# jnetter6/RRTQX_3D

Measured on NVIDIA B200. Metric: kd_range_queries_per_s, higher is better.
Workload: dtype f64

## Files before the change

### rrtqx_3d_b200/csrc/range_fused.cuh

```cuda

constexpr int FUSED_TAB = 256;
constexpr int FUSED_ROUNDS = 4;
#ifndef FUSED_U
#define FUSED_U 4
#endif

__device__ __forceinline__ void sts32(unsigned addr, int v) {
  asm volatile("st.shared.b32 [%0], %1;" ::"r"(addr), "r"(v) : "memory");
}
__device__ __forceinline__ int lds32(unsigned addr) {
  int v;
  asm volatile("ld.shared.b32 %0, [%1];" : "=r"(v) : "r"(addr) : "memory");
  return v;
}
__device__ __forceinline__ unsigned pin_reg(unsigned v) {
  unsigned r;
  asm volatile("mov.u32 %0, %1;" : "=r"(r) : "r"(v));
  return r;
}

#ifdef RRTQX_LEGACY
template <int D, int QN>
struct Group {
  double q[QN][D];
// ... 396 lines not shown
  const double *dT = nullptr;
  if (dr) {
    res->tq.ensure((size_t)nq, st);
    thresh_kernel<<<div_up(nq, 256), 256, 0, st>>>(dr, nq, res->tq.p);
    post_launch(ctx);
    dT = res->tq.p;
  }
  size_t cap = count_only ? 0 : res->idx.cap;
  if (!count_only && want_dist) cap = std::min(cap, res->dist.cap);
  if (!count_only && cap == 0) {
    cap = (size_t)nq * 64;
    res->idx.ensure(cap, st, 0, 1.0);
    if (want_dist) res->dist.ensure(cap, st, 0, 1.0);
    cap = want_dist ? std::min(res->idx.cap, res->dist.cap) : res->idx.cap;
  }
  double k_est = 1e9;
  if (!dr && r > 0.0 && std::isfinite(r)) {
    double vol = 1.0;
    int dims = 0;
    const int nd[3] = {t->nx, t->ny, t->nz};
    for (int c = 0; c < 3; ++c)
      if (nd[c] > 1) { vol *= nd[c] * t->cell[c]; dims++; }
    const double ball = dims == 3 ? 4.18879 * r * r * r : (dims == 2 ? 3.14159 * r * r : 2.0 * r);
    k_est = dims ? 1.15 * (double)t->n * ball / vol : (double)t->n;
  } else if (!dr) {
    k_est = 0.0;
  }
  int variant = k_est <= 576.0 ? 0 : (k_est <= 1280.0 ? 1 : (k_est <= 2048.0 ? 2 : 3));
  if (ctx->tune.fused_variant >= 0) variant = ctx->tune.fused_variant;
#ifdef RRTQX_LEGACY
  const int kernel_gen = ctx->tune.range_kernel;
#endif
  unsigned long long total = 0;
  for (int attempt = 0; attempt < 2; ++attempt) {
    GridView g = t->view();
    RQ_CUDA(cudaMemsetAsync(res->cursor.p, 0, 4 * sizeof(unsigned long long), st));
    {
      PhaseScope p2(ctx, "range_fill");
#ifdef RRTQX_LEGACY
#define RQ_FUSED(NW_, CAP_)                                                                                          \
  launch_fused<D, NW_, CAP_>(ctx, g, dq, res->qbins > 0 ? res->qsorted.p : nullptr, res->qorder.p, nq, r, T, dr, dT, res->counts.p, res->offsets.p, res->idx.p, \
                             want_dist ? res->dist.p : nullptr, (unsigned long long)cap, res->cursor.p,             \
                             count_only ? 0 : 1)
#endif
#define RQ_V5(NW_, CAP_, TAB_)                                                                                       \
  launch_v5<D, NW_, CAP_, TAB_>(ctx, g, kq, kqs, korder, knq, r, T, dr, dT, kcounts, koffsets, res->idx.p, \
                                want_dist ? res->dist.p : nullptr, (unsigned long long)cap, res->cursor.p, count_only ? 0 : 1, ghost ? 1 : 0)
#ifdef RRTQX_LEGACY
      if (kernel_gen >= 5 || ghost)
#endif
      {
        const int v5_nw = ctx->tune.v5_nw;
#ifdef RRTQX_EXPERIMENT
        if (variant == 0 && v5_nw == 32) RQ_V5(32, 704, 256);
        else
#endif
        if (variant == 0 && v5_nw == 28) RQ_V5(28, 704, 256);
        else if (variant == 0 && v5_nw == 20) RQ_V5(20, 704, 256);
        else if (variant == 0) RQ_V5(24, 704, 256);
        else if (variant == 1) RQ_V5(24, 1408, 512);
        else if (variant == 2) RQ_V5(16, 2176, 1024);
        else RQ_V5(8, 4224, 2048);
      }
#ifdef RRTQX_LEGACY
      else
      if (variant == 0) RQ_FUSED(28, 576);
      else if (variant == 1) RQ_FUSED(20, 1280);
      else if (variant == 2) RQ_FUSED(12, 2048);
      else RQ_FUSED(6, 4096);
#undef RQ_FUSED
#endif
#undef RQ_V5
    }
    RQ_CUDA(cudaMemcpyAsync(&total, res->cursor.p, sizeof(total), cudaMemcpyDeviceToHost, st));
    RQ_CUDA(cudaStreamSynchronize(st));
    if (count_only || total <= cap) break;
    RQ_REQUIRE(attempt == 0, "internal: range output did not fit after resizing");
    cap = (size_t)total + (size_t)(total / 32) + 1024;
    res->idx.ensure(cap, st, 0, 1.0);
    if (want_dist) res->dist.ensure(cap, st, 0, 1.0);
    cap = want_dist ? std::min(res->idx.cap, res->dist.cap) : res->idx.cap;
  }
  if (ghost) {
    ghost_merge_kernel<<<div_up(nq, 256), 256, 0, st>>>(res->vcounts.p, res->voffsets.p, nq, res->counts.p, res->offsets.p);
    post_launch(ctx);
  }
  res->n_queries = nq;
  res->total = (int64_t)total;
  res->has_lists = !count_only;
  res->has_dist = !count_only && want_dist;
}
```

### rrtqx_3d_b200/csrc/range_v5.cuh

```cuda

constexpr int V5_TABPAD = 16;
constexpr int V5_UNIT = 128;
constexpr int V5_RING = 64;
#ifndef V5_U_TRIPS
#define V5_U_TRIPS 4
#endif
constexpr int V5_U = V5_U_TRIPS;

__device__ __forceinline__ unsigned long long pk2(float a, float b) {
  unsigned long long r;
  asm("mov.b64 %0, {%1, %2};" : "=l"(r) : "f"(a), "f"(b));
  return r;
}
__device__ __forceinline__ void upk2(unsigned long long r, float &a, float &b) {
  asm("mov.b64 {%0, %1}, %2;" : "=f"(a), "=f"(b) : "l"(r));
}
__device__ __forceinline__ unsigned long long fma2(unsigned long long a, unsigned long long b, unsigned long long c) {
  unsigned long long r;
  asm("fma.rn.f32x2 %0, %1, %2, %3;" : "=l"(r) : "l"(a), "l"(b), "l"(c));
  return r;
}
__device__ __forceinline__ unsigned long long sub2(unsigned long long a, unsigned long long b) {
  unsigned long long r;
  asm("sub.rn.f32x2 %0, %1, %2;" : "=l"(r) : "l"(a), "l"(b));
// ... 67 lines not shown
  auto visit = [&](bool valid, int node, double px, double py, double pz, double pw) {
    const double s = sqdist<D>(q, px, py, pz, pw);
    const bool hit = valid && (s < T);
    const unsigned m = __ballot_sync(FULL, hit);
    if (WRITE && hit) {
      const int64_t o = base + cnt + __popc(m & lt);
      out_idx[o] = node;
      if (out_dist) out_dist[o] = __dsqrt_rn(s);
    }
    cnt += __popc(m);
  };
  if (g.n_sorted > 0 && r > 0.0) {
    const double r_infl = r * (1.0 + 1e-9);
    const double r2_infl = r_infl * r_infl;
    const int cy0 = cell_of(q[1] - r_infl, g.lo[1], g.inv[1], g.ny);
    const int cy1 = cell_of(q[1] + r_infl, g.lo[1], g.inv[1], g.ny);
    const int cz0 = D >= 3 ? cell_of(q[2] - r_infl, g.lo[2], g.inv[2], g.nz) : 0;
    const int cz1 = D >= 3 ? cell_of(q[2] + r_infl, g.lo[2], g.inv[2], g.nz) : 0;
    const int wy = cy1 - cy0 + 1;
    const int nrows = wy * (cz1 - cz0 + 1);
    for (int rb = 0; rb < nrows; rb += 32) {
      RowSpan sp{0, 0};
      const int row = rb + lane;
      if (row < nrows) sp = row_span<D>(g, q, r_infl, r2_infl, cy0 + row % wy, cz0 + row / wy);
      const int lim = min(32, nrows - rb);
      for (int t = 0; t < lim; ++t) {
        const int a = __shfl_sync(FULL, sp.start, t);
        const int b = __shfl_sync(FULL, sp.end, t);
        for (int j0 = a; j0 < b; j0 += 32) {
          const int j = j0 + lane;
          const bool v = j < b;
          double4 p = make_double4(0, 0, 0, 0);
          int node = 0;
          if (v) {
            p = g.d4[j];
            node = D <= 3 ? (int)__double_as_longlong(p.w) : g.sperm[j];
          }
          visit(v, node, p.x, p.y, p.z, p.w);
        }
      }
    }
  }
  if (r > 0.0)
    for (int j0 = g.n_sorted; j0 < g.n_total; j0 += 32) {
      const int j = j0 + lane;
      const bool v = j < g.n_total;
      double4 p = make_double4(0, 0, 0, 0);
      if (v) p = g.pos[j];
      visit(v, j, p.x, p.y, p.z, p.w);
    }
  return cnt;
}

template <int D, bool TAIL>
__device__ __forceinline__ void v5_flush(const GridView &g, const double *q, unsigned sbuf_k, unsigned stab, int n, int lane,
                                         int32_t *__restrict__ oi, double *__restrict__ od) {
#ifndef V5_FLUSH_U
#define V5_FLUSH_U 4
#endif
  constexpr int U = V5_FLUSH_U;
  auto fetch = [&](unsigned h, int &node, double4 &p) {
    if (!TAIL || !(h & 0x8000u)) {
      const int ent = lds32(stab + 4u * (h >> 3));
      const int slot = (ent >> 4) + (int)(h & 7u);
      p = ldg256(g.d4 + slot);
      node = D <= 3 ? (int)__double_as_longlong(p.w) : g.sperm[slot];
    } else {
      node = g.n_sorted + (int)(h & 0x7fffu);
      p = g.pos[node];
    }
  };
  const int n_full = (n / (32 * U)) * (32 * U);
  for (int h0 = lane; h0 < n_full; h0 += 32 * U) {
    int node[U];
    double4 p[U];
#pragma unroll
    for (int u = 0; u < U; ++u) fetch(lds16(sbuf_k + 2u * (unsigned)(h0 + 32 * u)), node[u], p[u]);
#pragma unroll
    for (int u = 0; u < U; ++u) {
      v5_st(oi + h0 + 32 * u, node[u]);
      if (od) v5_st(od + h0 + 32 * u, __dsqrt_rn(sqdist<D>(q, p[u].x, p[u].y, p[u].z, p[u].w)));
    }
  }
  auto tail = [&](auto rows_tag) {
    constexpr int R = decltype(rows_tag)::value;
    const int h0 = n_full + lane;
    int node[R];
    double4 p[R];
#pragma unroll
    for (int u = 0; u < R; ++u) {
      const int hh = h0 + 32 * u < n ? h0 + 32 * u : 0;
      fetch(lds16(sbuf_k + 2u * (unsigned)hh), node[u], p[u]);
    }
#pragma unroll
    for (int u = 0; u < R; ++u)
      if (h0 + 32 * u < n) {
        v5_st(oi + h0 + 32 * u, node[u]);
        if (od) v5_st(od + h0 + 32 * u, __dsqrt_rn(sqdist<D>(q, p[u].x, p[u].y, p[u].z, p[u].w)));
      }
  };
  const int rem = n - n_full;
  if (U >= 4 && rem > 64) tail(std::integral_constant<int, (U >= 4 ? 4 : 1)>{});
  else if (rem > 32) tail(std::integral_constant<int, 2>{});
  else if (rem > 0) tail(std::integral_constant<int, 1>{});
}

template <int D>
__device__ __noinline__ void v5_flush_tail(const GridView *gp, const double *qs, unsigned sbuf_k, unsigned stab, int n,
                                           int32_t *__restrict__ oi, double *__restrict__ od) {
  double q[D];
#pragma unroll
  for (int c = 0; c < D; ++c) q[c] = qs[c];
  v5_flush<D, true>(*gp, q, sbuf_k, stab, n, lane_id(), oi, od);
}

struct V5Radius {
  float rf, r2f;
  float Tm;
  float cM1, cM0;
  float sum_max;
  bool live;
};
__host__ __device__ __forceinline__ V5Radius v5_radius(double r, double T, bool have) {
  V5Radius R;
  R.live = have && (r > 0.0);
  const double ri = r * (1.0 + 1e-9);
  R.rf = f32_up(ri) * (1.0f + 1e-6f);
  R.r2f = f32_up(ri * ri) * (1.0f + 1e-5f);
  float Tm, M;
  bool ex;
  v5_filter(T, 0.0f, Tm, M, ex);
  const float Tf = f32_up(T), sT = sqrtf(Tf);
  R.Tm = Tm;
  R.cM0 = M;
  R.cM1 = 12.0f * (sT * 1.000001f) * 6.03e-8f * 1.000001f;
  R.sum_max = ex ? -1.0f : sT * 0.999999f * (1.0f / (1024.0f * 6.03e-8f)) * 0.99999f;
  if (!R.live) { R.Tm = -INFINITY; R.r2f = -1.0f; R.cM0 = 0.0f; R.cM1 = 0.0f; R.sum_max = INFINITY; }
  return R;
}

struct V5Params {
  V5Radius RU;
  float invx, invy, invz, celly, cellz;
  unsigned unit;
  int ghost_pairs;
};

__device__ __forceinline__ int clampi_fast(float v, int n) { return min(max(__float2int_rd(v), 0), n - 1); }

__device__ __forceinline__ float sqrt_approx(float x) {
  float y;
  asm("sqrt.approx.f32 %0, %1;" : "=f"(y) : "f"(x));
  return y;
}

template <int D, int NW, int CAP, int TAB, bool UNIFORM>
__global__ void __launch_bounds__(NW * 32, 1)
range_v5_kernel(GridView g_param, V5Params P, const double *__restrict__ queries, const double *__restrict__ qsorted,
                const int32_t *__restrict__ qorder, int64_t nq, double r_uniform, double T_uniform,
                const double *__restrict__ ranges, const double *__restrict__ Tq, int32_t *__restrict__ counts,
                int64_t *__restrict__ offsets, int32_t *__restrict__ out_idx, double *__restrict__ out_dist,
                unsigned long long cap, unsigned long long *__restrict__ cursor, int write_lists) {
  extern __shared__ int s_buf[];
  __shared__ GridView s_g;
  __shared__ unsigned s_ticket;
  __shared__ unsigned s_pub[V5_RING];
  __shared__ long long s_base[V5_RING];
  const GridView &g = g_param;
  if (threadIdx.x == 0) { s_g = g_param; s_ticket = 0; }
  if (threadIdx.x < V5_RING) s_pub[threadIdx.x] = 0;
  __syncthreads();
  const int lane = lane_id(), warp = threadIdx.x >> 5;
  const unsigned lt = lanemask_lt();
  const unsigned s0 = (unsigned)__cvta_generic_to_shared(s_buf);
  const unsigned sbuf = pin_reg(s0 + 2u * (unsigned)(warp * 2 * CAP));
  const unsigned stab = pin_reg(s0 + 2u * (unsigned)(NW * 2 * CAP) + 4u * (unsigned)(warp * (TAB + V5_TABPAD)));
  const float &invx = P.invx, &invy = P.invy, &invz = P.invz, &celly = P.celly, &cellz = P.cellz;
  const float fmaxabs = g.n_sorted > 0 ? *g.fmaxabs : 0.0f;
  const bool has_tail = g.n_total > g.n_sorted;
  const unsigned grp = pin_reg((unsigned)lane >> 3), sub = pin_reg((unsigned)lane & 7u);
  constexpr bool uniform = UNIFORM;

  const int64_t n_pairs = (nq + 1) >> 1;
  for (;;) {
    {
      unsigned tk = 0;
      if (lane == 0) tk = atomicAdd(&s_ticket, 1u);
      tk = __shfl_sync(FULL, tk, 0);
      const unsigned unit = tk / P.unit, off = tk - unit * P.unit, slot = unit % V5_RING;
      long long base = 0;
      if (lane == 0) {
        if (off == 0) {
          base = (long long)atomicAdd(&cursor[1], (unsigned long long)P.unit);
          s_base[slot] = base;
          __threadfence_block();
          atomicExch(&s_pub[slot], unit + 1u);
        } else {
          while (atomicAdd(&s_pub[slot], 0u) != unit + 1u) __nanosleep(32);
          base = *(volatile long long *)&s_base[slot];
        }
      }
      base = __shfl_sync(FULL, base, 0);
      if (base >= n_pairs) break;
      const int64_t qfirst = (base + off) * 2;
      if (qfirst >= nq) continue;
      const bool have1 = qfirst + 1 < nq;
      const int qid0 = qorder[qfirst], qid1 = have1 ? qorder[qfirst + 1] : -1;
      const double *qs0 = qsorted ? qsorted + qfirst * D : queries + (int64_t)qid0 * D;
      const double *qs1 = !have1 ? qs0 : (qsorted ? qs0 + D : queries + (int64_t)qid1 * D);
      V5Radius Rq0, Rq1;
      if (!uniform) {
        Rq0 = v5_radius(ranges[qid0], Tq[qid0], true);
        Rq1 = have1 ? v5_radius(ranges[qid1], Tq[qid1], true) : Rq0;
      }
      const V5Radius &R0 = uniform ? P.RU : Rq0, &R1 = uniform ? P.RU : Rq1;
      auto fp32_query = [&](const double *qs, float (&qf)[4], float &mab) {
        mab = 0.0f;
#pragma unroll
        for (int c = 0; c < 4; ++c) {
          if (c < D) {
            const double v = qs[c];
            qf[c] = __double2float_rn(c < 3 ? __dsub_rn(v, g.lo[c < 3 ? c : 0]) : v);
            mab = fmaxf(mab, fabsf(qf[c]));
          } else {
            qf[c] = 0.0f;
          }
        }
#pragma unroll
        for (int c = 0; c < D; ++c) if (qf[c] != qf[c]) mab = -1.0f;
      };
      auto exactT = [&](int k) { return uniform ? T_uniform : ((k == 0 || !have1) ? Tq[qid0] : Tq[qid1]); };
      auto exactR = [&](int k) { return uniform ? r_uniform : ((k == 0 || !have1) ? ranges[qid0] : ranges[qid1]); };

      int root_extra = 0;
      {
        const double4 p0 = g.pos[0];
        double q0[D], q1[D];
#pragma unroll
        for (int c = 0; c < D; ++c) { q0[c] = qs0[c]; q1[c] = qs1[c]; }
        const double T0 = exactT(0), T1 = exactT(1);
        const double sr0 = sqdist<D>(q0, p0.x, p0.y, p0.z, p0.w), sr1 = sqdist<D>(q1, p0.x, p0.y, p0.z, p0.w);
        if (!(sr0 < T0) && sr0 <= T0 * 1.000001 && __dsqrt_rn(sr0) <= exactR(0)) root_extra |= 1;
        if (have1 && !P.ghost_pairs && !(sr1 < T1) && sr1 <= T1 * 1.000001 && __dsqrt_rn(sr1) <= exactR(1)) root_extra |= 2;
      }
      const bool live0 = R0.live, live1 = R1.live;
      bool exact_path = false;
      int n_ent = 0;
      if (live0 || live1) {
        float qf0[4], qf1[4], mab0, mab1;
        fp32_query(qs0, qf0, mab0);
        fp32_query(qs1, qf1, mab1);
        const bool rows0 = live0 && !(mab0 < 0.0f), rows1 = live1 && !(mab1 < 0.0f);
        exact_path = (rows0 && !(fmaxabs + mab0 <= R0.sum_max)) || (rows1 && !(fmaxabs + mab1 <= R1.sum_max));
        if (!exact_path && g.n_sorted > 0 && (rows0 || rows1)) {
          float ff0[3], ff1[3];
          ff0[0] = qf0[0] * invx; ff0[1] = qf0[1] * invy; ff0[2] = D >= 3 ? qf0[2] * invz : 0.0f;
          ff1[0] = qf1[0] * invx; ff1[1] = qf1[1] * invy; ff1[2] = D >= 3 ? qf1[2] * invz : 0.0f;
          const float ry0 = R0.rf * invy + 1e-3f, ry1 = R1.rf * invy + 1e-3f;
          const float rz0 = R0.rf * invz + 1e-3f, rz1 = R1.rf * invz + 1e-3f;
          int cy0 = 0x7fffffff, cy1 = -1, cz0 = 0, cz1 = 0;
          if (D >= 3) { cz0 = 0x7fffffff; cz1 = -1; }
          if (rows0) {
            cy0 = clampi_fast(ff0[1] - ry0, g.ny); cy1 = clampi_fast(ff0[1] + ry0, g.ny);
            if (D >= 3) { cz0 = clampi_fast(ff0[2] - rz0, g.nz); cz1 = clampi_fast(ff0[2] + rz0, g.nz); }
          }
          if (rows1) {
            cy0 = min(cy0, clampi_fast(ff1[1] - ry1, g.ny)); cy1 = max(cy1, clampi_fast(ff1[1] + ry1, g.ny));
            if (D >= 3) { cz0 = min(cz0, clampi_fast(ff1[2] - rz1, g.nz)); cz1 = max(cz1, clampi_fast(ff1[2] + rz1, g.nz)); }
          }
          const int wy = cy1 - cy0 + 1;
          const int sh = 32 - __clz(wy - 1);
          const int nslots = (cz1 - cz0 + 1) << sh;
          for (int rb = 0; rb < nslots; rb += 32) {
            int sa_ = 0, sb_ = 0;
            const int slot = rb + lane;
            const int ry = slot & ((1 << sh) - 1);
            if (slot < nslots && ry < wy) {
              const int cy = cy0 + ry, cz = cz0 + (slot >> sh);
              const float ylo = cy == 0 ? -INFINITY : (float)cy, yhi = cy == g.ny - 1 ? INFINITY : (float)(cy + 1);
              const float zlo = cz == 0 ? -INFINITY : (float)cz, zhi = cz == g.nz - 1 ? INFINITY : (float)(cz + 1);
              int ca = 0x7fffffff, cb = -1;
              auto span = [&](const float *ff, float r2f) {
                float dy = fmaxf(fmaxf(ylo - ff[1], ff[1] - yhi) * (1.0f - 1e-6f) - 1e-3f, 0.0f) * celly;
                float rem = r2f - dy * dy;
                if (D >= 3) {
                  float dz = fmaxf(fmaxf(zlo - ff[2], ff[2] - zhi) * (1.0f - 1e-6f) - 1e-3f, 0.0f) * cellz;
                  rem -= dz * dz;
                }
                if (rem >= 0.0f) {
                  const float xc = sqrt_approx(rem) * (1.0f + 1e-5f) * invx + 1e-3f;
                  ca = min(ca, clampi_fast(ff[0] - xc, g.nx));
                  cb = max(cb, clampi_fast(ff[0] + xc, g.nx));
                }
              };
              if (rows0) span(ff0, R0.r2f);
              if (rows1) span(ff1, R1.r2f);
              if (cb >= ca) {
                const int rbase = (cz * g.ny + cy) * g.nx;
                sa_ = g.cell_start[rbase + ca];
                sb_ = g.cell_start[rbase + cb + 1];
              }
            }
            const int todo = (sb_ - sa_ + 7) >> 3;
            int incl = todo;
#pragma unroll
            for (int o = 1; o < 32; o <<= 1) {
              const int t = __shfl_up_sync(FULL, incl, o);
              if (lane >= o) incl += t;
            }
            const int sum = __shfl_sync(FULL, incl, 31);
            if (n_ent + sum > TAB) {
              exact_path = true;
              break;
            }
            unsigned ta = stab + 4u * (unsigned)(n_ent + incl - todo);
            for (int i = 0; i < todo; ++i) {
              sts32(ta, (sa_ << 4) | min(8, sb_ - sa_));
              ta += 4u;
              sa_ += 8;
            }
            n_ent += sum;
          }
        }
      }
      int cnt0 = 0, cnt1 = 0;
      bool overflow = false;
      if (exact_path) {
        cnt0 = live0 ? v5_exact_query<D, false>(&s_g, qs0, exactT(0), exactR(0), 0, nullptr, nullptr) : 0;
        cnt1 = (live1 && have1) ? v5_exact_query<D, false>(&s_g, qs1, exactT(1), exactR(1), 0, nullptr, nullptr) : 0;
        overflow = true;
      } else if (live0 || live1) {
        float qf0[4], qf1[4], mab0, mab1;
        fp32_query(qs0, qf0, mab0);
        fp32_query(qs1, qf1, mab1);
        const unsigned long long qx2 = pk2(qf0[0], qf1[0]), qy2 = pk2(qf0[1], qf1[1]);
        const unsigned long long qz2 = pk2(qf0[2], qf1[2]), qw2 = pk2(qf0[3], qf1[3]);
        const unsigned long long nT2 = pk2(-R0.Tm, -R1.Tm);
        const float M = fmaxf(R0.cM1 * (fmaxabs + mab0) + R0.cM0, R1.cM1 * (fmaxabs + mab1) + R1.cM0) * 1.000001f;
        unsigned wp0 = sbuf, wp1 = sbuf + 2u * CAP;
        const unsigned lim0 = sbuf + 2u * (CAP - 32 * V5_U), lim1 = sbuf + 2u * (2 * CAP - 32 * V5_U);

        const unsigned goff = 4u * grp;
        const unsigned hv0 = (grp << 3) | sub;
        int jj[V5_U];
        float4 c[V5_U];
        const int dummy = g.n_sorted + 7;
        auto load_group = [&](unsigned tb) {
          const unsigned taddr = tb + goff;
#pragma unroll
          for (int u = 0; u < V5_U; ++u) {
            const int ent = lds32(taddr + 16u * u);
            jj[u] = sub < (unsigned)(ent & 15) ? (ent >> 4) + (int)sub : dummy;
          }
#pragma unroll
          for (int u = 0; u < V5_U; ++u) {
            c[u] = g.f4[jj[u]];
          }
        };
        auto test_group = [&](auto store_tag, unsigned tb, bool more) {
          constexpr bool STORE = decltype(store_tag)::value;
          const unsigned hv = hv0 + ((tb - stab) << 1);
          float sa[V5_U], sb[V5_U];
          int jc[V5_U];
          float band = INFINITY;
#pragma unroll
          for (int u = 0; u < V5_U; ++u) {
            unsigned long long s2 = sub2(qx2, pk2(c[u].x, c[u].x));
            s2 = fma2(s2, s2, nT2);
            unsigned long long d2 = sub2(qy2, pk2(c[u].y, c[u].y));
            s2 = fma2(d2, d2, s2);
            if (D >= 3) { d2 = sub2(qz2, pk2(c[u].z, c[u].z)); s2 = fma2(d2, d2, s2); }
            if (D >= 4) { d2 = sub2(qw2, pk2(c[u].w, c[u].w)); s2 = fma2(d2, d2, s2); }
            upk2(s2, sa[u], sb[u]);
            band = fminf(band, fminf(fabsf(sa[u]), fabsf(sb[u])));
            jc[u] = jj[u];
          }
          if (more) load_group(tb + 4u * 4 * V5_U);
          if (__any_sync(FULL, band <= M)) {
            double qa[D], qb[D];
#pragma unroll
            for (int cc = 0; cc < D; ++cc) { qa[cc] = qs0[cc]; qb[cc] = qs1[cc]; }
            const double Ta = exactT(0), Tb = exactT(1);
#pragma unroll
            for (int u = 0; u < V5_U; ++u) {
              if (sa[u] < INFINITY || sb[u] < INFINITY) {
                const double4 p = g.d4[jc[u]];
                sa[u] = (live0 && sqdist<D>(qa, p.x, p.y, p.z, p.w) < Ta) ? -INFINITY : INFINITY;
                sb[u] = (live1 && sqdist<D>(qb, p.x, p.y, p.z, p.w) < Tb) ? -INFINITY : INFINITY;
              }
            }
          }
#pragma unroll
          for (int u = 0; u < V5_U; ++u) {
            const bool h0 = sa[u] < M;
            const unsigned m0 = __ballot_sync(FULL, h0);
            if (STORE && h0) sts16(wp0 + 2u * __popc(m0 & lt), hv + 32u * u);
            wp0 += 2u * __popc(m0);
            const bool h1 = sb[u] < M;
            const unsigned m1 = __ballot_sync(FULL, h1);
            if (STORE && h1) sts16(wp1 + 2u * __popc(m1 & lt), hv + 32u * u);
            wp1 += 2u * __popc(m1);
          }
        };
        if (n_ent > 0) {
          if (lane < V5_TABPAD) sts32(stab + 4u * (unsigned)(n_ent + lane), 0);
          __syncwarp();
          unsigned tb = stab;
          const unsigned tend = stab + 4u * (unsigned)n_ent;
          load_group(tb);
          while (tb < tend && wp0 <= lim0 && wp1 <= lim1) {
            const unsigned nb = tb + 4u * 4 * V5_U;
            test_group(std::true_type{}, tb, nb < tend);
            tb = nb;
          }
          if (tb < tend) {
            overflow = true;
            do {
              const unsigned nb = tb + 4u * 4 * V5_U;
              test_group(std::false_type{}, tb, nb < tend);
              tb = nb;
            } while (tb < tend);
          }
          __syncwarp();
        }
        if (has_tail && g.n_total - g.n_sorted > 0x8000) overflow = true;
        if (has_tail) {
          double qa[D], qb[D];
#pragma unroll
          for (int cc = 0; cc < D; ++cc) { qa[cc] = qs0[cc]; qb[cc] = qs1[cc]; }
          const double Ta = exactT(0), Tb = exactT(1);
          for (int j0 = g.n_sorted; j0 < g.n_total; j0 += 32) {
            const int j = j0 + lane;
            const bool v = j < g.n_total;
            double4 p = make_double4(0, 0, 0, 0);
            if (v) p = g.pos[j];
            const bool h0 = v && live0 && (sqdist<D>(qa, p.x, p.y, p.z, p.w) < Ta);
            const bool h1 = v && live1 && (sqdist<D>(qb, p.x, p.y, p.z, p.w) < Tb);
            const unsigned m0 = __ballot_sync(FULL, h0);
            const unsigned o0 = wp0 + 2u * __popc(m0 & lt);
            if (h0 && o0 < sbuf + 2u * CAP) sts16(o0, 0x8000u | (unsigned)((j - g.n_sorted) & 0x7fff));
            wp0 += 2u * __popc(m0);
            const unsigned m1 = __ballot_sync(FULL, h1);
            const unsigned o1 = wp1 + 2u * __popc(m1 & lt);
            if (h1 && o1 < sbuf + 4u * CAP) sts16(o1, 0x8000u | (unsigned)((j - g.n_sorted) & 0x7fff));
            wp1 += 2u * __popc(m1);
          }
        }
        cnt0 = (int)((wp0 - sbuf) >> 1);
        cnt1 = (int)((wp1 - (sbuf + 2u * CAP)) >> 1);
        if (cnt0 > CAP || cnt1 > CAP) overflow = true;
      }
      const bool live1w = live1 && have1;
      if (!have1) cnt1 = 0;

      const int tot0 = cnt0 + (root_extra & 1), tot1 = cnt1 + ((root_extra >> 1) & 1);
      unsigned long long b0 = 0;
      if (lane == 0) b0 = atomicAdd(&cursor[0], (unsigned long long)(tot0 + tot1));
      b0 = __shfl_sync(FULL, b0, 0);
      if (lane == 0) {
        counts[qid0] = tot0;
        offsets[qid0] = (int64_t)b0;
        if (have1) {
          counts[qid1] = tot1;
          offsets[qid1] = (int64_t)(b0 + (unsigned long long)tot0);
        }
      }
      if (!write_lists || b0 + (unsigned long long)(tot0 + tot1) > cap) continue;
      __syncwarp();
      auto emit = [&](int k, const double *qs, int cnt, int64_t base, bool live_k) {
        if (!live_k) return;
        if (overflow) {
          v5_exact_query<D, true>(&s_g, qs, exactT(k), exactR(k), base, out_idx, out_dist);
        } else {
          const unsigned sb_k = sbuf + 2u * (unsigned)(k * CAP);
          if (has_tail) {
            v5_flush_tail<D>(&s_g, qs, sb_k, stab, cnt, out_idx + base, out_dist ? out_dist + base : nullptr);
          } else {
            double q[D];
#pragma unroll
            for (int c = 0; c < D; ++c) q[c] = qs[c];
            v5_flush<D, false>(g, q, sb_k, stab, cnt, lane, out_idx + base, out_dist ? out_dist + base : nullptr);
          }
        }
      };
#pragma unroll 1
      for (int k = 0; k < 2; ++k)
        emit(k, k ? qs1 : qs0, k ? cnt1 : cnt0, (int64_t)b0 + (k ? tot0 : 0), k ? live1w : live0);
      if (root_extra && lane == 0) {
        const double4 p0 = g.pos[0];
        if (root_extra & 1) {
          double q[D];
#pragma unroll
          for (int c = 0; c < D; ++c) q[c] = qs0[c];
          out_idx[b0 + cnt0] = 0;
          if (out_dist) out_dist[b0 + cnt0] = __dsqrt_rn(sqdist<D>(q, p0.x, p0.y, p0.z, p0.w));
        }
        if (root_extra & 2) {
          double q[D];
#pragma unroll
          for (int c = 0; c < D; ++c) q[c] = qs1[c];
          out_idx[b0 + tot0 + cnt1] = 0;
          if (out_dist) out_dist[b0 + tot0 + cnt1] = __dsqrt_rn(sqdist<D>(q, p0.x, p0.y, p0.z, p0.w));
        }
      }
      __syncwarp();
    }
  }
}

template <int D>
__global__ void ghost_expand_kernel(WrapInfo wrap, const double *__restrict__ queries, const double *__restrict__ qsorted,
                                    const int32_t *__restrict__ qorder, int64_t nq, double r,
                                    double *__restrict__ vq, int32_t *__restrict__ vorder) {
  const int64_t j = (int64_t)blockIdx.x * blockDim.x + threadIdx.x;
  if (j >= nq) return;
  const int qid = qorder[j];
  const double *src = qsorted ? qsorted + j * D : queries + (int64_t)qid * D;
  double q[D], gh[D];
#pragma unroll
  for (int k = 0; k < D; ++k) q[k] = src[k];
  const bool used = make_ghost<D>(wrap, q, 1, r, gh);
#pragma unroll
  for (int k = 0; k < D; ++k) {
    vq[(2 * j) * D + k] = q[k];
    vq[(2 * j + 1) * D + k] = used ? gh[k] : __longlong_as_double(0x7ff8000000000000LL);
  }
  vorder[2 * j] = 2 * qid;
  vorder[2 * j + 1] = 2 * qid + 1;
}
__global__ void ghost_merge_kernel(const int32_t *__restrict__ vcounts, const int64_t *__restrict__ voffsets, int64_t nq,
                                   int32_t *__restrict__ counts, int64_t *__restrict__ offsets) {
  const int64_t q = (int64_t)blockIdx.x * blockDim.x + threadIdx.x;
  if (q >= nq) return;
  counts[q] = vcounts[2 * q] + vcounts[2 * q + 1];
  offsets[q] = voffsets[2 * q];
}

template <int D, int NW, int CAP, int TAB>
static void launch_v5(rrtqx_ctx *ctx, const GridView &g, const double *dq, const double *dqs, const int32_t *qorder,
                      int64_t nq, double r, double T, const double *dr, const double *dT, int32_t *counts,
                      int64_t *offsets, int32_t *idx, double *dist, unsigned long long cap, unsigned long long *cursor,
                      int write_lists, int ghost_pairs = 0) {
  const size_t smem = (size_t)NW * (CAP + TAB + V5_TABPAD) * sizeof(int);
  if (ctx->smem_attr_done.insert((const void *)range_v5_kernel<D, NW, CAP, TAB, true>).second) {
    RQ_CUDA(cudaFuncSetAttribute(range_v5_kernel<D, NW, CAP, TAB, true>, cudaFuncAttributeMaxDynamicSharedMemorySize, (int)smem));
    RQ_CUDA(cudaFuncSetAttribute(range_v5_kernel<D, NW, CAP, TAB, false>, cudaFuncAttributeMaxDynamicSharedMemorySize, (int)smem));
  }
  V5Params P;
  P.RU = v5_radius(r, T, true);
  P.invx = (float)g.inv[0]; P.invy = (float)g.inv[1]; P.invz = (float)g.inv[2];
  P.celly = (float)g.cell[1]; P.cellz = (float)g.cell[2];
  P.unit = ctx->tune.v5_unit ? ctx->tune.v5_unit : (unsigned)V5_UNIT;
  P.ghost_pairs = ghost_pairs;
  const int64_t n_units = ((nq + 1) / 2 + P.unit - 1) / P.unit;
  const int blocks = (int)std::max<int64_t>(1, std::min<int64_t>(n_units, (int64_t)ctx->sm_count));
  if (dr)
    range_v5_kernel<D, NW, CAP, TAB, false><<<blocks, NW * 32, smem, ctx->stream>>>(g, P, dq, dqs, qorder, nq, r, T, dr, dT, counts,
                                                                              offsets, idx, dist, cap, cursor, write_lists);
  else
    range_v5_kernel<D, NW, CAP, TAB, true><<<blocks, NW * 32, smem, ctx->stream>>>(g, P, dq, dqs, qorder, nq, r, T, dr, dT, counts,
                                                                             offsets, idx, dist, cap, cursor, write_lists);
  post_launch(ctx);
}
```

Baseline: 359.5 million.

## Store paired-query hits as one shared union list with per-query hit flags

Replaces the two per-query shared-memory hit lists with one union list. Codes hit by both queries are written from the front and codes hit by only one are written from the back, each tagged with 14-bit flags. The flush step fetches each shared candidate point once and emits it for both queries, computing output offsets with ballots. This cuts duplicate global point loads and shared-memory writes for overlapping queries. In exchange it shrinks the code space to 14 bits, adds extra ballots and divergence in flush, and adds an optional debug counter.

```diff
diff --git a/rrtqx_3d_b200/csrc/range_fused.cuh b/rrtqx_3d_b200/csrc/range_fused.cuh
--- a/rrtqx_3d_b200/csrc/range_fused.cuh
+++ b/rrtqx_3d_b200/csrc/range_fused.cuh
@@ -494,6 +494,14 @@
     }
     RQ_CUDA(cudaMemcpyAsync(&total, res->cursor.p, sizeof(total), cudaMemcpyDeviceToHost, st));
     RQ_CUDA(cudaStreamSynchronize(st));
+#ifdef V5_COUNT_UNION
+    {
+      unsigned long long uc[2];
+      RQ_CUDA(cudaMemcpy(uc, res->cursor.p + 2, sizeof(uc), cudaMemcpyDeviceToHost));
+      fprintf(stderr, "v5 union list: %llu codes for %llu per-query hits (ratio to one query's hits %.4f)\n", uc[0], uc[1],
+              uc[1] ? 2.0 * (double)uc[0] / (double)uc[1] : 0.0);
+    }
+#endif
     if (count_only || total <= cap) break;
     RQ_REQUIRE(attempt == 0, "internal: range output did not fit after resizing");
     cap = (size_t)total + (size_t)(total / 32) + 1024;
diff --git a/rrtqx_3d_b200/csrc/range_v5.cuh b/rrtqx_3d_b200/csrc/range_v5.cuh
--- a/rrtqx_3d_b200/csrc/range_v5.cuh
+++ b/rrtqx_3d_b200/csrc/range_v5.cuh
@@ -143,66 +143,77 @@
   return cnt;
 }
 
+constexpr unsigned V5_HIT0 = 0x4000u, V5_HIT1 = 0x8000u, V5_CODE = 0x3fffu, V5_BOTH = V5_HIT0 | V5_HIT1;
+
 template <int D, bool TAIL>
-__device__ __forceinline__ void v5_flush(const GridView &g, const double *q, unsigned sbuf_k, unsigned stab, int n, int lane,
-                                         int32_t *__restrict__ oi, double *__restrict__ od) {
+__device__ __forceinline__ void v5_flush(const GridView &g, const double (&q0)[D], const double (&q1)[D], unsigned sbuf,
+                                         unsigned stab, int n, int tail_lo, int tail_hi, bool pair_list, int w0, int w1,
+                                         int lane, unsigned lt, int32_t *__restrict__ oi, double *__restrict__ od) {
 #ifndef V5_FLUSH_U
 #define V5_FLUSH_U 4
 #endif
   constexpr int U = V5_FLUSH_U;
-  auto fetch = [&](unsigned h, int &node, double4 &p) {
-    if (!TAIL || !(h & 0x8000u)) {
-      const int ent = lds32(stab + 4u * (h >> 3));
+  auto fetch = [&](unsigned h, int i, int &node, double4 &p) {
+    if (!TAIL || i < tail_lo || i >= tail_hi) {
+      const int ent = lds32(stab + 4u * ((h & V5_CODE) >> 3));
       const int slot = (ent >> 4) + (int)(h & 7u);
       p = ldg256(g.d4 + slot);
       node = D <= 3 ? (int)__double_as_longlong(p.w) : g.sperm[slot];
     } else {
-      node = g.n_sorted + (int)(h & 0x7fffu);
+      node = g.n_sorted + (int)(h & V5_CODE);
       p = g.pos[node];
     }
   };
-  const int n_full = (n / (32 * U)) * (32 * U);
-  for (int h0 = lane; h0 < n_full; h0 += 32 * U) {
-    int node[U];
-    double4 p[U];
-#pragma unroll
-    for (int u = 0; u < U; ++u) fetch(lds16(sbuf_k + 2u * (unsigned)(h0 + 32 * u)), node[u], p[u]);
-#pragma unroll
-    for (int u = 0; u < U; ++u) {
-      v5_st(oi + h0 + 32 * u, node[u]);
-      if (od) v5_st(od + h0 + 32 * u, __dsqrt_rn(sqdist<D>(q, p[u].x, p[u].y, p[u].z, p[u].w)));
-    }
-  }
-  auto tail = [&](auto rows_tag) {
+  auto step = [&](auto rows_tag, int h0) {
     constexpr int R = decltype(rows_tag)::value;
-    const int h0 = n_full + lane;
+    unsigned c[R];
     int node[R];
     double4 p[R];
 #pragma unroll
     for (int u = 0; u < R; ++u) {
-      const int hh = h0 + 32 * u < n ? h0 + 32 * u : 0;
-      fetch(lds16(sbuf_k + 2u * (unsigned)hh), node[u], p[u]);
+      const bool v = h0 + 32 * u < n;
+      const int hh = v ? h0 + 32 * u : 0;
+      c[u] = lds16(sbuf + 2u * (unsigned)hh);
+      fetch(c[u], hh, node[u], p[u]);
+      if (!v) c[u] = 0;
     }
 #pragma unroll
-    for (int u = 0; u < R; ++u)
-      if (h0 + 32 * u < n) {
-        v5_st(oi + h0 + 32 * u, node[u]);
-        if (od) v5_st(od + h0 + 32 * u, __dsqrt_rn(sqdist<D>(q, p[u].x, p[u].y, p[u].z, p[u].w)));
-      }
+    for (int u = 0; u < R; ++u) {
+      const unsigned m0 = __ballot_sync(FULL, c[u] & V5_HIT0), m1 = __ballot_sync(FULL, c[u] & V5_HIT1);
+      const int o0 = w0 + __popc(m0 & lt), o1 = w1 + __popc(m1 & lt);
+      w0 += __popc(m0);
+      w1 += __popc(m1);
+      const bool first0 = c[u] & V5_HIT0;
+      if (c[u] != 0) {
+        double q[D];
+#pragma unroll
+        for (int k = 0; k < D; ++k) q[k] = first0 ? q0[k] : q1[k];
+        const int o = first0 ? o0 : o1;
+        v5_st(oi + o, node[u]);
+        if (od) v5_st(od + o, __dsqrt_rn(sqdist<D>(q, p[u].x, p[u].y, p[u].z, p[u].w)));
+        if (pair_list) {
+          v5_st(oi + o1, node[u]);
+          if (od) v5_st(od + o1, __dsqrt_rn(sqdist<D>(q1, p[u].x, p[u].y, p[u].z, p[u].w)));
+        }
+      }
+    }
   };
+  const int n_full = (n / (32 * U)) * (32 * U);
+  for (int h0 = lane; h0 < n_full; h0 += 32 * U) step(std::integral_constant<int, U>{}, h0);
   const int rem = n - n_full;
-  if (U >= 4 && rem > 64) tail(std::integral_constant<int, (U >= 4 ? 4 : 1)>{});
-  else if (rem > 32) tail(std::integral_constant<int, 2>{});
-  else if (rem > 0) tail(std::integral_constant<int, 1>{});
+  if (U >= 4 && rem > 64) step(std::integral_constant<int, (U >= 4 ? 4 : 1)>{}, n_full + lane);
+  else if (rem > 32) step(std::integral_constant<int, 2>{}, n_full + lane);
+  else if (rem > 0) step(std::integral_constant<int, 1>{}, n_full + lane);
 }
 
 template <int D>
-__device__ __noinline__ void v5_flush_tail(const GridView *gp, const double *qs, unsigned sbuf_k, unsigned stab, int n,
+__device__ __noinline__ void v5_flush_tail(const GridView *gp, const double *qs0, const double *qs1, unsigned sbuf,
+                                           unsigned stab, int n, int tail_lo, int tail_hi, bool pair_list, int w0, int w1,
                                            int32_t *__restrict__ oi, double *__restrict__ od) {
-  double q[D];
-#pragma unroll
-  for (int c = 0; c < D; ++c) q[c] = qs[c];
-  v5_flush<D, true>(*gp, q, sbuf_k, stab, n, lane_id(), oi, od);
+  double q0[D], q1[D];
+#pragma unroll
+  for (int c = 0; c < D; ++c) { q0[c] = qs0[c]; q1[c] = qs1[c]; }
+  v5_flush<D, true>(*gp, q0, q1, sbuf, stab, n, tail_lo, tail_hi, pair_list, w0, w1, lane_id(), lanemask_lt(), oi, od);
 }
 
 struct V5Radius {
@@ -252,6 +263,7 @@
                 const double *__restrict__ ranges, const double *__restrict__ Tq, int32_t *__restrict__ counts,
                 int64_t *__restrict__ offsets, int32_t *__restrict__ out_idx, double *__restrict__ out_dist,
                 unsigned long long cap, unsigned long long *__restrict__ cursor, int write_lists) {
+  static_assert(TAB * 8 <= (int)V5_CODE + 1, "table hit codes must fit 14 bits");
   extern __shared__ int s_buf[];
   __shared__ GridView s_g;
   __shared__ unsigned s_ticket;
@@ -334,7 +346,7 @@
         if (!(sr0 < T0) && sr0 <= T0 * 1.000001 && __dsqrt_rn(sr0) <= exactR(0)) root_extra |= 1;
         if (have1 && !P.ghost_pairs && !(sr1 < T1) && sr1 <= T1 * 1.000001 && __dsqrt_rn(sr1) <= exactR(1)) root_extra |= 2;
       }
-      const bool live0 = R0.live, live1 = R1.live;
+      const bool live0 = R0.live, live1 = R1.live && have1;
       bool exact_path = false;
       int n_ent = 0;
       if (live0 || live1) {
@@ -415,10 +427,12 @@
         }
       }
       int cnt0 = 0, cnt1 = 0;
+      int n_pair = 0, n_one = 0;
+      int n_pair_tab = 0, n_one_tab = 0;
       bool overflow = false;
       if (exact_path) {
         cnt0 = live0 ? v5_exact_query<D, false>(&s_g, qs0, exactT(0), exactR(0), 0, nullptr, nullptr) : 0;
-        cnt1 = (live1 && have1) ? v5_exact_query<D, false>(&s_g, qs1, exactT(1), exactR(1), 0, nullptr, nullptr) : 0;
+        cnt1 = live1 ? v5_exact_query<D, false>(&s_g, qs1, exactT(1), exactR(1), 0, nullptr, nullptr) : 0;
         overflow = true;
       } else if (live0 || live1) {
         float qf0[4], qf1[4], mab0, mab1;
@@ -426,10 +440,10 @@
         fp32_query(qs1, qf1, mab1);
         const unsigned long long qx2 = pk2(qf0[0], qf1[0]), qy2 = pk2(qf0[1], qf1[1]);
         const unsigned long long qz2 = pk2(qf0[2], qf1[2]), qw2 = pk2(qf0[3], qf1[3]);
-        const unsigned long long nT2 = pk2(-R0.Tm, -R1.Tm);
+        const unsigned long long nT2 = pk2(-R0.Tm, live1 ? -R1.Tm : INFINITY);
         const float M = fmaxf(R0.cM1 * (fmaxabs + mab0) + R0.cM0, R1.cM1 * (fmaxabs + mab1) + R1.cM0) * 1.000001f;
-        unsigned wp0 = sbuf, wp1 = sbuf + 2u * CAP;
-        const unsigned lim0 = sbuf + 2u * (CAP - 32 * V5_U), lim1 = sbuf + 2u * (2 * CAP - 32 * V5_U);
+        unsigned wb = sbuf, ws = sbuf + 4u * CAP;
+        int n1 = 0;
 
         const unsigned goff = 4u * grp;
         const unsigned hv0 = (grp << 3) | sub;
@@ -483,14 +497,13 @@
           }
 #pragma unroll
           for (int u = 0; u < V5_U; ++u) {
-            const bool h0 = sa[u] < M;
-            const unsigned m0 = __ballot_sync(FULL, h0);
-            if (STORE && h0) sts16(wp0 + 2u * __popc(m0 & lt), hv + 32u * u);
-            wp0 += 2u * __popc(m0);
-            const bool h1 = sb[u] < M;
-            const unsigned m1 = __ballot_sync(FULL, h1);
-            if (STORE && h1) sts16(wp1 + 2u * __popc(m1 & lt), hv + 32u * u);
-            wp1 += 2u * __popc(m1);
+            const bool h0 = sa[u] < M, h1 = sb[u] < M;
+            const unsigned mb = __ballot_sync(FULL, h0 && h1), ms = __ballot_sync(FULL, h0 != h1);
+            if (STORE && h0 && h1) sts16(wb + 2u * __popc(mb & lt), (hv + 32u * u) | V5_BOTH);
+            if (STORE && h0 != h1) sts16(ws - 2u - 2u * __popc(ms & lt), (hv + 32u * u) | (h0 ? V5_HIT0 : V5_HIT1));
+            wb += 2u * __popc(mb);
+            ws -= 2u * __popc(ms);
+            n1 += h1 && !h0;
           }
         };
         if (n_ent > 0) {
@@ -499,7 +512,7 @@
           unsigned tb = stab;
           const unsigned tend = stab + 4u * (unsigned)n_ent;
           load_group(tb);
-          while (tb < tend && wp0 <= lim0 && wp1 <= lim1) {
+          while (tb < tend && (int)(ws - wb) >= 2 * 32 * V5_U) {
             const unsigned nb = tb + 4u * 4 * V5_U;
             test_group(std::true_type{}, tb, nb < tend);
             tb = nb;
@@ -514,7 +527,9 @@
           }
           __syncwarp();
         }
-        if (has_tail && g.n_total - g.n_sorted > 0x8000) overflow = true;
+        n_pair_tab = (int)((wb - sbuf) >> 1);
+        n_one_tab = (int)((sbuf + 4u * CAP - ws) >> 1);
+        if (has_tail && g.n_total - g.n_sorted > (int)V5_CODE + 1) overflow = true;
         if (has_tail) {
           double qa[D], qb[D];
 #pragma unroll
@@ -527,22 +542,30 @@
             if (v) p = g.pos[j];
             const bool h0 = v && live0 && (sqdist<D>(qa, p.x, p.y, p.z, p.w) < Ta);
             const bool h1 = v && live1 && (sqdist<D>(qb, p.x, p.y, p.z, p.w) < Tb);
-            const unsigned m0 = __ballot_sync(FULL, h0);
-            const unsigned o0 = wp0 + 2u * __popc(m0 & lt);
-            if (h0 && o0 < sbuf + 2u * CAP) sts16(o0, 0x8000u | (unsigned)((j - g.n_sorted) & 0x7fff));
-            wp0 += 2u * __popc(m0);
-            const unsigned m1 = __ballot_sync(FULL, h1);
-            const unsigned o1 = wp1 + 2u * __popc(m1 & lt);
-            if (h1 && o1 < sbuf + 4u * CAP) sts16(o1, 0x8000u | (unsigned)((j - g.n_sorted) & 0x7fff));
-            wp1 += 2u * __popc(m1);
-          }
-        }
-        cnt0 = (int)((wp0 - sbuf) >> 1);
-        cnt1 = (int)((wp1 - (sbuf + 2u * CAP)) >> 1);
-        if (cnt0 > CAP || cnt1 > CAP) overflow = true;
-      }
-      const bool live1w = live1 && have1;
-      if (!have1) cnt1 = 0;
+            const unsigned mb = __ballot_sync(FULL, h0 && h1), ms = __ballot_sync(FULL, h0 != h1);
+            const unsigned code = ((unsigned)(j - g.n_sorted) & V5_CODE) | (h0 ? V5_HIT0 : 0u) | (h1 ? V5_HIT1 : 0u);
+            if ((int)(ws - wb) >= 2 * (__popc(mb) + __popc(ms))) {
+              if (h0 && h1) sts16(wb + 2u * __popc(mb & lt), code);
+              if (h0 != h1) sts16(ws - 2u - 2u * __popc(ms & lt), code);
+            }
+            wb += 2u * __popc(mb);
+            ws -= 2u * __popc(ms);
+            n1 += h1 && !h0;
+          }
+        }
+        n_pair = (int)((wb - sbuf) >> 1);
+        n_one = (int)((sbuf + 4u * CAP - ws) >> 1);
+        const int n_one1 = __reduce_add_sync(FULL, n1);
+        cnt0 = n_pair + n_one - n_one1;
+        cnt1 = n_pair + n_one1;
+        if (n_pair + n_one > 2 * CAP) overflow = true;
+#ifdef V5_COUNT_UNION
+        if (lane == 0 && !overflow) {
+          atomicAdd(&cursor[2], (unsigned long long)(n_pair + n_one));
+          atomicAdd(&cursor[3], (unsigned long long)(cnt0 + cnt1));
+        }
+#endif
+      }
 
       const int tot0 = cnt0 + (root_extra & 1), tot1 = cnt1 + ((root_extra >> 1) & 1);
       unsigned long long b0 = 0;
@@ -558,25 +581,31 @@
       }
       if (!write_lists || b0 + (unsigned long long)(tot0 + tot1) > cap) continue;
       __syncwarp();
-      auto emit = [&](int k, const double *qs, int cnt, int64_t base, bool live_k) {
-        if (!live_k) return;
-        if (overflow) {
-          v5_exact_query<D, true>(&s_g, qs, exactT(k), exactR(k), base, out_idx, out_dist);
-        } else {
-          const unsigned sb_k = sbuf + 2u * (unsigned)(k * CAP);
+      if (overflow) {
+#pragma unroll 1
+        for (int k = 0; k < 2; ++k)
+          if (k ? live1 : live0)
+            v5_exact_query<D, true>(&s_g, k ? qs1 : qs0, exactT(k), exactR(k), (int64_t)b0 + (k ? tot0 : 0), out_idx, out_dist);
+      } else {
+#pragma unroll 1
+        for (int k = 0; k < 2; ++k) {
+          const unsigned base = k ? sbuf + 4u * CAP - 2u * (unsigned)n_one : sbuf;
+          const int n = k ? n_one : n_pair;
+          const int tail_lo = k ? 0 : n_pair_tab, tail_hi = k ? n_one - n_one_tab : n_pair;
+          const int w0 = k ? n_pair : 0, w1 = tot0 + (k ? n_pair : 0);
+          if (n == 0) continue;
           if (has_tail) {
-            v5_flush_tail<D>(&s_g, qs, sb_k, stab, cnt, out_idx + base, out_dist ? out_dist + base : nullptr);
+            v5_flush_tail<D>(&s_g, qs0, qs1, base, stab, n, tail_lo, tail_hi, k == 0, w0, w1, out_idx + b0,
+                             out_dist ? out_dist + b0 : nullptr);
           } else {
-            double q[D];
-#pragma unroll
-            for (int c = 0; c < D; ++c) q[c] = qs[c];
-            v5_flush<D, false>(g, q, sb_k, stab, cnt, lane, out_idx + base, out_dist ? out_dist + base : nullptr);
-          }
-        }
-      };
-#pragma unroll 1
-      for (int k = 0; k < 2; ++k)
-        emit(k, k ? qs1 : qs0, k ? cnt1 : cnt0, (int64_t)b0 + (k ? tot0 : 0), k ? live1w : live0);
+            double q0[D], q1[D];
+#pragma unroll
+            for (int c = 0; c < D; ++c) { q0[c] = qs0[c]; q1[c] = qs1[c]; }
+            v5_flush<D, false>(g, q0, q1, base, stab, n, 0, 0, k == 0, w0, w1, lane, lt, out_idx + b0,
+                               out_dist ? out_dist + b0 : nullptr);
+          }
+        }
+      }
       if (root_extra && lane == 0) {
         const double4 p0 = g.pos[0];
         if (root_extra & 1) {
```

After: 196.7 million (median of 6 runs). 45.3% lower.

## Merge paired-query candidate lists into one shared buffer with hit bits

Applied to the files above, without the earlier changes.

Each warp now keeps one union candidate list for its two queries instead of two separate lists. Every entry carries two hit bits saying which query matched, and the flush pass fetches each candidate point once and emits it for one or both queries using ballot-based compaction. The aim is to cut duplicate global point loads and shared-memory traffic for candidates common to both queries, and CAP is raised to fit the larger union list. In exchange, the flush becomes more divergent with extra ballots per row, tail entries must recompute distances for both queries, and table codes are limited to 14 bits.

```diff
diff --git a/rrtqx_3d_b200/csrc/range_fused.cuh b/rrtqx_3d_b200/csrc/range_fused.cuh
--- a/rrtqx_3d_b200/csrc/range_fused.cuh
+++ b/rrtqx_3d_b200/csrc/range_fused.cuh
@@ -472,15 +472,15 @@
       {
         const int v5_nw = ctx->tune.v5_nw;
 #ifdef RRTQX_EXPERIMENT
-        if (variant == 0 && v5_nw == 32) RQ_V5(32, 704, 256);
+        if (variant == 0 && v5_nw == 32) RQ_V5(32, 1024, 256);
         else
 #endif
-        if (variant == 0 && v5_nw == 28) RQ_V5(28, 704, 256);
-        else if (variant == 0 && v5_nw == 20) RQ_V5(20, 704, 256);
-        else if (variant == 0) RQ_V5(24, 704, 256);
-        else if (variant == 1) RQ_V5(24, 1408, 512);
-        else if (variant == 2) RQ_V5(16, 2176, 1024);
-        else RQ_V5(8, 4224, 2048);
+        if (variant == 0 && v5_nw == 28) RQ_V5(28, 1024, 256);
+        else if (variant == 0 && v5_nw == 20) RQ_V5(20, 1024, 256);
+        else if (variant == 0) RQ_V5(24, 1024, 256);
+        else if (variant == 1) RQ_V5(24, 2816, 512);
+        else if (variant == 2) RQ_V5(16, 4352, 1024);
+        else RQ_V5(8, 8448, 2048);
       }
 #ifdef RRTQX_LEGACY
       else
diff --git a/rrtqx_3d_b200/csrc/range_v5.cuh b/rrtqx_3d_b200/csrc/range_v5.cuh
--- a/rrtqx_3d_b200/csrc/range_v5.cuh
+++ b/rrtqx_3d_b200/csrc/range_v5.cuh
@@ -143,52 +143,85 @@
   return cnt;
 }
 
+constexpr unsigned V5_HIT0 = 0x4000u, V5_HIT1 = 0x8000u;
+constexpr int V5_MAX_TAIL = 0x10000;
+
 template <int D, bool TAIL>
-__device__ __forceinline__ void v5_flush(const GridView &g, const double *q, unsigned sbuf_k, unsigned stab, int n, int lane,
-                                         int32_t *__restrict__ oi, double *__restrict__ od) {
+__device__ __forceinline__ void v5_flush(const GridView &g, const double *qs0, const double *qs1, unsigned sbuf,
+                                         unsigned stab, int n, int n_tab, unsigned live, double T0, double T1,
+                                         int32_t *__restrict__ out_idx, double *__restrict__ out_dist, int64_t w0,
+                                         int64_t w1) {
 #ifndef V5_FLUSH_U
 #define V5_FLUSH_U 4
 #endif
   constexpr int U = V5_FLUSH_U;
-  auto fetch = [&](unsigned h, int &node, double4 &p) {
-    if (!TAIL || !(h & 0x8000u)) {
-      const int ent = lds32(stab + 4u * (h >> 3));
-      const int slot = (ent >> 4) + (int)(h & 7u);
+  const int lane = lane_id();
+  const unsigned lt = lanemask_lt();
+  auto fetch = [&](int h, int &node, double4 &p, unsigned &mem) {
+    const unsigned c = lds16(sbuf + 2u * (unsigned)h);
+    if (!TAIL || h < n_tab) {
+      const int ent = lds32(stab + 4u * ((c & 0x3fffu) >> 3));
+      const int slot = (ent >> 4) + (int)(c & 7u);
       p = ldg256(g.d4 + slot);
       node = D <= 3 ? (int)__double_as_longlong(p.w) : g.sperm[slot];
+      mem = c >> 14;
     } else {
-      node = g.n_sorted + (int)(h & 0x7fffu);
+      node = g.n_sorted + (int)c;
       p = g.pos[node];
-    }
+      mem = 4u;
+    }
+  };
+  double q0[D], q1[D];
+#pragma unroll
+  for (int c = 0; c < D; ++c) { q0[c] = qs0[c]; q1[c] = qs1[c]; }
+  auto emit = [&](bool valid, int node, const double4 &p, unsigned mem) {
+    bool h0 = mem & 1u, h1 = mem & 2u;
+    if (TAIL && mem == 4u) { h0 = sqdist<D>(q0, p.x, p.y, p.z, p.w) < T0; h1 = sqdist<D>(q1, p.x, p.y, p.z, p.w) < T1; }
+    h0 = h0 && valid && (live & 1u);
+    h1 = h1 && valid && (live & 2u);
+    const unsigned m0 = __ballot_sync(FULL, h0), m1 = __ballot_sync(FULL, h1);
+    if (h0) {
+      const int64_t o = w0 + __popc(m0 & lt);
+      v5_st(out_idx + o, node);
+      if (out_dist) v5_st(out_dist + o, __dsqrt_rn(sqdist<D>(q0, p.x, p.y, p.z, p.w)));
+    }
+    if (h1) {
+      const int64_t o = w1 + __popc(m1 & lt);
+      v5_st(out_idx + o, node);
+      if (out_dist) v5_st(out_dist + o, __dsqrt_rn(sqdist<D>(q1, p.x, p.y, p.z, p.w)));
+    }
+    w0 += __popc(m0);
+    w1 += __popc(m1);
   };
   const int n_full = (n / (32 * U)) * (32 * U);
   for (int h0 = lane; h0 < n_full; h0 += 32 * U) {
     int node[U];
     double4 p[U];
-#pragma unroll
-    for (int u = 0; u < U; ++u) fetch(lds16(sbuf_k + 2u * (unsigned)(h0 + 32 * u)), node[u], p[u]);
+    unsigned mem = 0;
 #pragma unroll
     for (int u = 0; u < U; ++u) {
-      v5_st(oi + h0 + 32 * u, node[u]);
-      if (od) v5_st(od + h0 + 32 * u, __dsqrt_rn(sqdist<D>(q, p[u].x, p[u].y, p[u].z, p[u].w)));
-    }
+      unsigned m;
+      fetch(h0 + 32 * u, node[u], p[u], m);
+      mem |= m << (3 * u);
+    }
+#pragma unroll
+    for (int u = 0; u < U; ++u) emit(true, node[u], p[u], (mem >> (3 * u)) & 7u);
   }
   auto tail = [&](auto rows_tag) {
     constexpr int R = decltype(rows_tag)::value;
     const int h0 = n_full + lane;
     int node[R];
     double4 p[R];
+    unsigned mem = 0;
 #pragma unroll
     for (int u = 0; u < R; ++u) {
       const int hh = h0 + 32 * u < n ? h0 + 32 * u : 0;
-      fetch(lds16(sbuf_k + 2u * (unsigned)hh), node[u], p[u]);
-    }
-#pragma unroll
-    for (int u = 0; u < R; ++u)
-      if (h0 + 32 * u < n) {
-        v5_st(oi + h0 + 32 * u, node[u]);
-        if (od) v5_st(od + h0 + 32 * u, __dsqrt_rn(sqdist<D>(q, p[u].x, p[u].y, p[u].z, p[u].w)));
-      }
+      unsigned m;
+      fetch(hh, node[u], p[u], m);
+      mem |= m << (3 * u);
+    }
+#pragma unroll
+    for (int u = 0; u < R; ++u) emit(h0 + 32 * u < n, node[u], p[u], (mem >> (3 * u)) & 7u);
   };
   const int rem = n - n_full;
   if (U >= 4 && rem > 64) tail(std::integral_constant<int, (U >= 4 ? 4 : 1)>{});
@@ -197,12 +230,11 @@
 }
 
 template <int D>
-__device__ __noinline__ void v5_flush_tail(const GridView *gp, const double *qs, unsigned sbuf_k, unsigned stab, int n,
-                                           int32_t *__restrict__ oi, double *__restrict__ od) {
-  double q[D];
-#pragma unroll
-  for (int c = 0; c < D; ++c) q[c] = qs[c];
-  v5_flush<D, true>(*gp, q, sbuf_k, stab, n, lane_id(), oi, od);
+__device__ __noinline__ void v5_flush_tail(const GridView *gp, const double *qs0, const double *qs1, unsigned sbuf,
+                                           unsigned stab, int n, int n_tab, unsigned live, double T0, double T1,
+                                           int32_t *__restrict__ out_idx, double *__restrict__ out_dist, int64_t w0,
+                                           int64_t w1) {
+  v5_flush<D, true>(*gp, qs0, qs1, sbuf, stab, n, n_tab, live, T0, T1, out_idx, out_dist, w0, w1);
 }
 
 struct V5Radius {
@@ -264,8 +296,9 @@
   const int lane = lane_id(), warp = threadIdx.x >> 5;
   const unsigned lt = lanemask_lt();
   const unsigned s0 = (unsigned)__cvta_generic_to_shared(s_buf);
-  const unsigned sbuf = pin_reg(s0 + 2u * (unsigned)(warp * 2 * CAP));
-  const unsigned stab = pin_reg(s0 + 2u * (unsigned)(NW * 2 * CAP) + 4u * (unsigned)(warp * (TAB + V5_TABPAD)));
+  static_assert(CAP % 2 == 0 && TAB <= 2048, "octet tables need 4-byte alignment; table codes have 14 bits");
+  const unsigned sbuf = pin_reg(s0 + 2u * (unsigned)(warp * CAP));
+  const unsigned stab = pin_reg(s0 + 2u * (unsigned)(NW * CAP) + 4u * (unsigned)(warp * (TAB + V5_TABPAD)));
   const float &invx = P.invx, &invy = P.invy, &invz = P.invz, &celly = P.celly, &cellz = P.cellz;
   const float fmaxabs = g.n_sorted > 0 ? *g.fmaxabs : 0.0f;
   const bool has_tail = g.n_total > g.n_sorted;
@@ -415,6 +448,7 @@
         }
       }
       int cnt0 = 0, cnt1 = 0;
+      int n_un = 0, n_tab = 0;
       bool overflow = false;
       if (exact_path) {
         cnt0 = live0 ? v5_exact_query<D, false>(&s_g, qs0, exactT(0), exactR(0), 0, nullptr, nullptr) : 0;
@@ -428,8 +462,8 @@
         const unsigned long long qz2 = pk2(qf0[2], qf1[2]), qw2 = pk2(qf0[3], qf1[3]);
         const unsigned long long nT2 = pk2(-R0.Tm, -R1.Tm);
         const float M = fmaxf(R0.cM1 * (fmaxabs + mab0) + R0.cM0, R1.cM1 * (fmaxabs + mab1) + R1.cM0) * 1.000001f;
-        unsigned wp0 = sbuf, wp1 = sbuf + 2u * CAP;
-        const unsigned lim0 = sbuf + 2u * (CAP - 32 * V5_U), lim1 = sbuf + 2u * (2 * CAP - 32 * V5_U);
+        unsigned wp = sbuf;
+        const unsigned lim = sbuf + 2u * (CAP - 32 * V5_U);
 
         const unsigned goff = 4u * grp;
         const unsigned hv0 = (grp << 3) | sub;
@@ -483,14 +517,13 @@
           }
 #pragma unroll
           for (int u = 0; u < V5_U; ++u) {
-            const bool h0 = sa[u] < M;
-            const unsigned m0 = __ballot_sync(FULL, h0);
-            if (STORE && h0) sts16(wp0 + 2u * __popc(m0 & lt), hv + 32u * u);
-            wp0 += 2u * __popc(m0);
-            const bool h1 = sb[u] < M;
-            const unsigned m1 = __ballot_sync(FULL, h1);
-            if (STORE && h1) sts16(wp1 + 2u * __popc(m1 & lt), hv + 32u * u);
-            wp1 += 2u * __popc(m1);
+            const bool h0 = sa[u] < M, h1 = sb[u] < M;
+            const unsigned m0 = __ballot_sync(FULL, h0), m1 = __ballot_sync(FULL, h1), m = m0 | m1;
+            if (STORE && (h0 || h1))
+              sts16(wp + 2u * __popc(m & lt), (hv + 32u * u) | (h0 ? V5_HIT0 : 0u) | (h1 ? V5_HIT1 : 0u));
+            wp += 2u * __popc(m);
+            cnt0 += __popc(m0);
+            cnt1 += __popc(m1);
           }
         };
         if (n_ent > 0) {
@@ -499,7 +532,7 @@
           unsigned tb = stab;
           const unsigned tend = stab + 4u * (unsigned)n_ent;
           load_group(tb);
-          while (tb < tend && wp0 <= lim0 && wp1 <= lim1) {
+          while (tb < tend && wp <= lim) {
             const unsigned nb = tb + 4u * 4 * V5_U;
             test_group(std::true_type{}, tb, nb < tend);
             tb = nb;
@@ -514,7 +547,8 @@
           }
           __syncwarp();
         }
-        if (has_tail && g.n_total - g.n_sorted > 0x8000) overflow = true;
+        n_tab = (int)((wp - sbuf) >> 1);
+        if (has_tail && g.n_total - g.n_sorted > V5_MAX_TAIL) overflow = true;
         if (has_tail) {
           double qa[D], qb[D];
 #pragma unroll
@@ -527,19 +561,16 @@
             if (v) p = g.pos[j];
             const bool h0 = v && live0 && (sqdist<D>(qa, p.x, p.y, p.z, p.w) < Ta);
             const bool h1 = v && live1 && (sqdist<D>(qb, p.x, p.y, p.z, p.w) < Tb);
-            const unsigned m0 = __ballot_sync(FULL, h0);
-            const unsigned o0 = wp0 + 2u * __popc(m0 & lt);
-            if (h0 && o0 < sbuf + 2u * CAP) sts16(o0, 0x8000u | (unsigned)((j - g.n_sorted) & 0x7fff));
-            wp0 += 2u * __popc(m0);
-            const unsigned m1 = __ballot_sync(FULL, h1);
-            const unsigned o1 = wp1 + 2u * __popc(m1 & lt);
-            if (h1 && o1 < sbuf + 4u * CAP) sts16(o1, 0x8000u | (unsigned)((j - g.n_sorted) & 0x7fff));
-            wp1 += 2u * __popc(m1);
-          }
-        }
-        cnt0 = (int)((wp0 - sbuf) >> 1);
-        cnt1 = (int)((wp1 - (sbuf + 2u * CAP)) >> 1);
-        if (cnt0 > CAP || cnt1 > CAP) overflow = true;
+            const unsigned m0 = __ballot_sync(FULL, h0), m1 = __ballot_sync(FULL, h1), m = m0 | m1;
+            const unsigned o = wp + 2u * __popc(m & lt);
+            if ((h0 || h1) && o < sbuf + 2u * CAP) sts16(o, (unsigned)(j - g.n_sorted) & 0xffffu);
+            wp += 2u * __popc(m);
+            cnt0 += __popc(m0);
+            cnt1 += __popc(m1);
+          }
+        }
+        n_un = (int)((wp - sbuf) >> 1);
+        if (n_un > CAP) overflow = true;
       }
       const bool live1w = live1 && have1;
       if (!have1) cnt1 = 0;
@@ -558,25 +589,6 @@
       }
       if (!write_lists || b0 + (unsigned long long)(tot0 + tot1) > cap) continue;
       __syncwarp();
-      auto emit = [&](int k, const double *qs, int cnt, int64_t base, bool live_k) {
-        if (!live_k) return;
-        if (overflow) {
-          v5_exact_query<D, true>(&s_g, qs, exactT(k), exactR(k), base, out_idx, out_dist);
-        } else {
-          const unsigned sb_k = sbuf + 2u * (unsigned)(k * CAP);
-          if (has_tail) {
-            v5_flush_tail<D>(&s_g, qs, sb_k, stab, cnt, out_idx + base, out_dist ? out_dist + base : nullptr);
-          } else {
-            double q[D];
-#pragma unroll
-            for (int c = 0; c < D; ++c) q[c] = qs[c];
-            v5_flush<D, false>(g, q, sb_k, stab, cnt, lane, out_idx + base, out_dist ? out_dist + base : nullptr);
-          }
-        }
-      };
-#pragma unroll 1
-      for (int k = 0; k < 2; ++k)
-        emit(k, k ? qs1 : qs0, k ? cnt1 : cnt0, (int64_t)b0 + (k ? tot0 : 0), k ? live1w : live0);
       if (root_extra && lane == 0) {
         const double4 p0 = g.pos[0];
         if (root_extra & 1) {
@@ -593,6 +605,20 @@
           out_idx[b0 + tot0 + cnt1] = 0;
           if (out_dist) out_dist[b0 + tot0 + cnt1] = __dsqrt_rn(sqdist<D>(q, p0.x, p0.y, p0.z, p0.w));
         }
+      }
+      if (overflow) {
+#pragma unroll 1
+        for (int k = 0; k < 2; ++k)
+          if (k ? live1w : live0)
+            v5_exact_query<D, true>(&s_g, k ? qs1 : qs0, exactT(k), exactR(k), (int64_t)b0 + (k ? tot0 : 0), out_idx, out_dist);
+      } else {
+        const unsigned live = (live0 ? 1u : 0u) | (live1w ? 2u : 0u);
+        if (has_tail)
+          v5_flush_tail<D>(&s_g, qs0, qs1, sbuf, stab, n_un, n_tab, live, exactT(0), exactT(1), out_idx, out_dist,
+                           (int64_t)b0, (int64_t)b0 + tot0);
+        else
+          v5_flush<D, false>(g, qs0, qs1, sbuf, stab, n_un, n_un, live, 0.0, 0.0, out_idx, out_dist, (int64_t)b0,
+                             (int64_t)b0 + tot0);
       }
       __syncwarp();
     }
@@ -632,7 +658,7 @@
                       int64_t nq, double r, double T, const double *dr, const double *dT, int32_t *counts,
                       int64_t *offsets, int32_t *idx, double *dist, unsigned long long cap, unsigned long long *cursor,
                       int write_lists, int ghost_pairs = 0) {
-  const size_t smem = (size_t)NW * (CAP + TAB + V5_TABPAD) * sizeof(int);
+  const size_t smem = (size_t)NW * (2 * CAP + 4 * (TAB + V5_TABPAD));
   if (ctx->smem_attr_done.insert((const void *)range_v5_kernel<D, NW, CAP, TAB, true>).second) {
     RQ_CUDA(cudaFuncSetAttribute(range_v5_kernel<D, NW, CAP, TAB, true>, cudaFuncAttributeMaxDynamicSharedMemorySize, (int)smem));
     RQ_CUDA(cudaFuncSetAttribute(range_v5_kernel<D, NW, CAP, TAB, false>, cudaFuncAttributeMaxDynamicSharedMemorySize, (int)smem));
```

After: 357.8 million before, 282.2 million after, median of 6. 21.1% lower.
